# rakeshvar/theanet

Hardware: AMD Instinct MI355X
Metric: training images/sec (fwd+bwd+update) MNIST-CNN bs4096, 1/2/4/8 MI355X (higher is better)
Workload: dtype f32; 1 GPU; params/mnist.prms 28x28x1 synthetic, global batch 4096 = 4096 images/GPU/step x 1, elastic stage on; global_batch=4096, parallelism=dp1, schedule=two steps in flight (exact: the update applies the old velocity)

## Files before the change

theanet_amd/csrc/convblock_mfma.hip:

```cpp
#include "common.h"

int tn_conv_wgrad_finish(tn_ctx* ctx, const float* partial, const float* dbpartial, float* dW,
                         float* db, int nblk, int K, int C, int f);

typedef float f32x4 __attribute__((ext_vector_type(4)));

#define CM_XR 12

struct CmGeom {
    int N, H, Wd, K, pad, Ho, Wo, Hp, Wp;
    int Wx, xplane;
    int xf;
    int PT;
    int npixp;
    int dzf;
    int tabf;
    int wavef;
    int dbg;
};

__device__ __forceinline__ void cm_wave_sync() {
    __builtin_amdgcn_fence(__ATOMIC_ACQ_REL, "wavefront");
    __builtin_amdgcn_wave_barrier();
}

__device__ __forceinline__ f32x4 cm_mfma(float a, float b, f32x4 c) {
    return __builtin_amdgcn_mfma_f32_16x16x4f32(a, b, c, 0, 0, 0);
}

template <int N>
__device__ __forceinline__ float cm_shr(float v) {
    return __int_as_float(__builtin_amdgcn_update_dpp(0, __float_as_int(v), 0x110 + N, 0xf, 0xf, false));
}

__device__ __forceinline__ int cm_div(int n, float rd) { return __float2int_rz(((float)n + .5f) * rd); }

template <int ACT>
__device__ __forceinline__ float cm_act(float z, int act, float prm) {
    if (ACT == TN_ACT_LEAKY) return fmaxf(0.f, z) + fminf(0.f, z) * prm;
    return tn_act_fwd(z, act, prm);
}
template <int ACT>
__device__ __forceinline__ float cm_actg(float a, int act, float prm) {
    if (ACT == TN_ACT_LEAKY) return a > 0.f ? 1.f : (a < 0.f ? prm : (prm > 0.f ? 1.f + prm : 0.f));
    return tn_act_grad_from_out(a, act, prm);
}

template <int C, int KS2, int ACT>
__global__ __launch_bounds__(256, 2) void convblock_bwd_mfma(
    const float* __restrict__ x, const float* __restrict__ W, const float* __restrict__ b,
    const float* __restrict__ g, float* __restrict__ dx, float* __restrict__ partial,
    float* __restrict__ dbpartial, CmGeom q, int act, float prm, float* __restrict__ tdbg) {
    constexpr int F = 3, FF = 9, CKK = C * FF;
    constexpr int KS1 = (CKK + 3) / 4;
    constexpr int NT = (CKK + 16) / 16;
    constexpr int NKT = (KS2 + 3) / 4;
    constexpr int NTD = 3;
    extern __shared__ __attribute__((aligned(16))) float sm[];
    const int lane = threadIdx.x & 63, wv = threadIdx.x >> 6;
    const int lo = lane & 15, qd = lane >> 4;
    const long long t0_ = __builtin_readcyclecounter();
    int ts_ = 0;
#define CM_STAMP() if (tdbg && blockIdx.x == (q.dbg >> 8) && threadIdx.x == 0 && ts_ < 20) tdbg[ts_++] = (float)(__builtin_readcyclecounter() - t0_)
    const int K = q.K, HW = q.H * q.Wd, CHW = C * HW, HpWp = q.Hp * q.Wp, KHW = K * HpWp;

    const int gw = blockIdx.x * 4 + wv, nw = gridDim.x * 4;
    float xr[CM_XR], gr[CM_XR];
#define CM_PREFETCH(N_)                                                                     \
    {                                                                                       \
        const float* xp_ = x + (size_t)(N_) * CHW;                                          \
        const float* gp_ = g + (size_t)(N_) * KHW;                                          \
        _Pragma("unroll") for (int j = 0; j < CM_XR; ++j) {                                 \
            xr[j] = xp_[min(lane + 64 * j, CHW - 1)];                                       \
            gr[j] = gp_[min(lane + 64 * j, KHW - 1)];                                       \
        }                                                                                   \
    }
    int n = __builtin_amdgcn_readfirstlane(gw);
    if (n < q.N) CM_PREFETCH(n);

    int* wtab = reinterpret_cast<int*>(sm);
    float* wbase = sm + q.tabf + wv * q.wavef;
    float* sx = wbase;
    float* sdx = sx + q.xf;
    float* sg = sdx;
    float* sdz = sdx + q.xf;
    const int ZERO = q.xf - 4, ONE = q.xf - 3;
    const int DUMMY = q.xf - 2;

    for (int i = threadIdx.x; i < 4 * q.PT; i += 256) {
        int e = 0;
        if (i < HpWp) {
            const int wy = i / q.Wp, wx = i - wy * q.Wp;
            const bool vx = 2 * wx + 1 < q.Wo, vy = 2 * wy + 1 < q.Ho;
            e = ((2 * wy * q.Wx + 2 * wx) << 4) | 1 | (vx ? 2 : 0) | (vy ? 4 : 0) | (vx && vy ? 8 : 0);
        }
        wtab[i] = e;
    }
    for (int i = lane * 4; i < q.xf; i += 256) *reinterpret_cast<float4*>(sx + i) = make_float4(0.f, 0.f, 0.f, 0.f);
    for (int i = lane; i < 4 * KS2 * 4; i += 64) sdz[(i >> 2) * q.npixp + 16 * q.PT + (i & 3)] = 0.f;
    for (int i = K * q.npixp + lane; i < q.dzf; i += 64) sdz[i] = 0.f;
    CM_STAMP();
    __syncthreads();
    CM_STAMP();
    if (lane == 0) sx[ONE] = 1.f;

    auto ckk_off = [&](int ckk) {
        const int c = ckk / FF, ab = ckk - c * FF, a = ab / F, bb = ab - a * F;
        return c * q.xplane + a * q.Wx + bb;
    };
    auto wf = [&](int k, int c, int ab) -> float {
        const bool ok = k < K && c < C && ab < FF;
        const float v = W[((size_t)min(k, K - 1) * C + min(c, C - 1)) * FF + (FF - 1 - min(ab, FF - 1))];
        return ok ? v : 0.f;
    };
    float Bw1[NKT][KS1];
    int off1[KS1];
#pragma unroll
    for (int s = 0; s < KS1; ++s) {
        const int ckk = 4 * s + qd;
        off1[s] = ckk < CKK ? ckk_off(ckk) : 0;
#pragma unroll
        for (int kt = 0; kt < NKT; ++kt) Bw1[kt][s] = wf(16 * kt + lo, ckk < CKK ? ckk / FF : C, ckk % FF);
    }
    int off3[NT], msk3[NT];
#pragma unroll
    for (int nt = 0; nt < NT; ++nt) {
        const int ckk = 16 * nt + lo;
        off3[nt] = ckk < CKK ? ckk_off(ckk) : (ckk == CKK ? ONE : ZERO);
        msk3[nt] = ckk < CKK ? -1 : 0;
    }
    float Aw2[NTD][KS2];
#pragma unroll
    for (int mt = 0; mt < NTD; ++mt)
#pragma unroll
        for (int s = 0; s < KS2; ++s) Aw2[mt][s] = wf(4 * s + qd, lo >> 2, 4 * mt + (lo & 3));
    float bk[NKT];
#pragma unroll
    for (int kt = 0; kt < NKT; ++kt) bk[kt] = b[min(16 * kt + lo, K - 1)];
    int tabr[CM_XR];
    const float rHW = __builtin_amdgcn_rcpf((float)HW), rWd = __builtin_amdgcn_rcpf((float)q.Wd);
#pragma unroll
    for (int j = 0; j < CM_XR; ++j) {
        const int i = min(lane + 64 * j, CHW - 1);
        const int c = cm_div(i, rHW), r = i - c * HW, y = cm_div(r, rWd), xx = r - y * q.Wd;
        tabr[j] = (lane + 64 * j < CHW) ? c * q.xplane + (y + q.pad) * q.Wx + xx + q.pad : DUMMY;
    }
    CM_STAMP();
    __builtin_amdgcn_s_waitcnt(0x0f70);
    CM_STAMP();
#pragma unroll
    for (int s = 0; s < KS1; ++s)
#pragma unroll
        for (int kt = 0; kt < NKT; ++kt) asm volatile("" : "+v"(Bw1[kt][s]));
#pragma unroll
    for (int mt = 0; mt < NTD; ++mt)
#pragma unroll
        for (int s = 0; s < KS2; ++s) asm volatile("" : "+v"(Aw2[mt][s]));
#pragma unroll
    for (int kt = 0; kt < NKT; ++kt) asm volatile("" : "+v"(bk[kt]));

    f32x4 accW[NKT][NT];
#pragma unroll
    for (int kt = 0; kt < NKT; ++kt)
#pragma unroll
        for (int nt = 0; nt < NT; ++nt) accW[kt][nt] = f32x4{0.f, 0.f, 0.f, 0.f};
    CM_STAMP();

    const int dyo = ((lo >> 1) & 1) * q.Wx + (lo & 1);
    const float tie = prm > 0.f ? 1.f + prm : 0.f;
    const int dcol = lo < q.Wo ? 4 * (lo >> 1) + (lo & 1) : 16 * q.PT;
    const int dmsk = lo < q.Wo ? -1 : 0;
    for (; n < q.N; n += nw) {
#pragma unroll
        for (int j = 0; j < CM_XR; ++j) {
            sx[tabr[j]] = xr[j];
            sg[min(lane + 64 * j, KHW - 1)] = gr[j];
        }
        if (n + nw < q.N) CM_PREFETCH(n + nw);
        cm_wave_sync();
        CM_STAMP();
        float av[KS1];
        {
            const int poff = (wtab[lo >> 2] >> 4) + dyo;
#pragma unroll
            for (int s = 0; s < KS1; ++s) av[s] = sx[poff + off1[s]];
        }
#pragma unroll 1
        for (int t = 0; t < q.PT; ++t) {
            f32x4 z[NKT];
#pragma unroll
            for (int kt = 0; kt < NKT; ++kt) z[kt] = f32x4{0.f, 0.f, 0.f, 0.f};
            if (!(q.dbg & 8)) {
#pragma unroll
            for (int s = 0; s < KS1; ++s)
#pragma unroll
                for (int kt = 0; kt < NKT; ++kt) z[kt] = cm_mfma(av[s], Bw1[kt][s], z[kt]);
            }
            {
                const int tn = min(t + 1, q.PT - 1);
                const int poff = (wtab[4 * tn + (lo >> 2)] >> 4) + dyo;
#pragma unroll
                for (int s = 0; s < KS1; ++s) av[s] = sx[poff + off1[s]];
            }
            const int wi = 4 * t + qd;
            const int e2 = wtab[wi];
            const int woff = e2 >> 4;
            float bv[4][NT];
#pragma unroll
            for (int r = 0; r < 4; ++r) {
                const int pw = woff + (r >> 1) * q.Wx + (r & 1);
#pragma unroll
                for (int nt = 0; nt < NT; ++nt) bv[r][nt] = sx[off3[nt] + (pw & msk3[nt])];
            }
            float dzv[NKT][4];
#pragma unroll
            for (int kt = 0; kt < NKT; ++kt) {
                const int k = 16 * kt + lo;
                float gv = sg[min(k, K - 1) * HpWp + min(wi, HpWp - 1)];
                gv = k < K ? gv : 0.f;
                float a[4];
                float m = -INFINITY;
#pragma unroll
                for (int r = 0; r < 4; ++r) {
                    a[r] = cm_act<ACT>(z[kt][r] + bk[kt], act, prm);
                    m = (e2 >> r & 1) ? fmaxf(m, a[r]) : m;
                }
#pragma unroll
                for (int r = 0; r < 4; ++r) {
                    float gp;
                    if (ACT == TN_ACT_LEAKY) {
                        gp = a[r] < 0.f ? prm : tie;
                        gp = a[r] > 0.f ? 1.f : gp;
                    } else {
                        gp = tn_act_grad_from_out(a[r], act, prm);
                    }
                    const float sel = ((e2 >> r & 1) && a[r] == m) ? gv : 0.f;
                    dzv[kt][r] = sel * gp;
                }
                if (k < K)
                    *reinterpret_cast<float4*>(sdz + k * q.npixp + 16 * t + 4 * qd) =
                        make_float4(dzv[kt][0], dzv[kt][1], dzv[kt][2], dzv[kt][3]);
            }
            if (!(q.dbg & 1)) {
#pragma unroll
            for (int r = 0; r < 4; ++r)
#pragma unroll
                for (int kt = 0; kt < NKT; ++kt)
#pragma unroll
                    for (int nt = 0; nt < NT; ++nt)
                        accW[kt][nt] = cm_mfma(dzv[kt][r], bv[r][nt], accW[kt][nt]);
            }
        }
        CM_STAMP();
        if (dx && !(q.dbg & 2)) {
            cm_wave_sync();
            float R1 = 0.f, R2 = 0.f;
            float* dxo = sdx + qd * q.xplane + lo;
            const bool dlive = (qd < C) && (lo < q.Wo + 2);
            float bcur[KS2];
            {
                const float* dzp = sdz + qd * q.npixp + dcol;
#pragma unroll
                for (int s = 0; s < KS2; ++s) bcur[s] = dzp[4 * s * q.npixp];
            }
#pragma unroll 1
            for (int y = 0; y < q.Ho; ++y) {
                const int yn = min(y + 1, q.Ho - 1);
                const int prow = 4 * (yn >> 1) * q.Wp + 2 * (yn & 1);
                const float* dzp = sdz + qd * q.npixp + dcol + (prow & dmsk);
                float bnxt[KS2];
#pragma unroll
                for (int s = 0; s < KS2; ++s) bnxt[s] = dzp[4 * s * q.npixp];
                f32x4 T[NTD];
#pragma unroll
                for (int mt = 0; mt < NTD; ++mt) T[mt] = f32x4{0.f, 0.f, 0.f, 0.f};
#pragma unroll
                for (int s = 0; s < KS2; ++s)
#pragma unroll
                    for (int mt = 0; mt < NTD; ++mt) T[mt] = cm_mfma(Aw2[mt][s], bcur[s], T[mt]);
#pragma unroll
                for (int s = 0; s < KS2; ++s) bcur[s] = bnxt[s];
                const float S0 = T[0][0] + cm_shr<1>(T[0][1]) + cm_shr<2>(T[0][2]);
                const float S1 = T[0][3] + cm_shr<1>(T[1][0]) + cm_shr<2>(T[1][1]);
                const float S2 = T[1][2] + cm_shr<1>(T[1][3]) + cm_shr<2>(T[2][0]);
                const float out = S0 + R1;
                R1 = S1 + R2;
                R2 = S2;
                if (dlive) dxo[y * q.Wx] = out;
            }
            if (dlive) {
                dxo[q.Ho * q.Wx] = R1;
                dxo[(q.Ho + 1) * q.Wx] = R2;
            }
            cm_wave_sync();
            float* dxp = dx + (size_t)n * CHW;
#pragma unroll
            for (int j = 0; j < CM_XR; ++j) {
                const int i = lane + 64 * j;
                if (i < CHW) dxp[i] = sdx[tabr[j]];
            }
        }
        cm_wave_sync();
        CM_STAMP();
    }
#undef CM_PREFETCH
    __syncthreads();
#pragma unroll
    for (int kt = 0; kt < NKT; ++kt)
#pragma unroll
        for (int nt = 0; nt < NT; ++nt)
#pragma unroll
            for (int r = 0; r < 4; ++r) wbase[((kt * NT + nt) * 4 + r) * 64 + lane] = accW[kt][nt][r];
    __syncthreads();
    for (int e = threadIdx.x; e < K * (CKK + 1); e += 256) {
        const int k = e / (CKK + 1), ckk = e - k * (CKK + 1);
        const int idx = (((k >> 4) * NT + (ckk >> 4)) * 4 + (k & 3)) * 64 + ((k & 15) >> 2) * 16 + (ckk & 15);
        const float* src = sm + q.tabf + idx;
        const float s = ((src[0] + src[q.wavef]) + src[2 * q.wavef]) + src[3 * q.wavef];
        if (ckk < CKK)
            partial[(size_t)blockIdx.x * K * CKK + k * CKK + ckk] = s;
        else
            dbpartial[(size_t)blockIdx.x * K + k] = s;
    }
    CM_STAMP();
#undef CM_STAMP
}

template <int C, int KS2, int ACT, bool W44>
__global__ __launch_bounds__(256, 2) void convblock_bwd_mask_mfma(
    const float* __restrict__ x, const float* __restrict__ W, const float* __restrict__ g,
    const float* __restrict__ y, const uint8_t* __restrict__ mask, float* __restrict__ dx,
    float* __restrict__ partial, float* __restrict__ dbpartial, CmGeom q, int act, float prm,
    float* __restrict__ tdbg) {
    constexpr int F = 3, FF = 9, CKK = C * FF;
    constexpr int NKT = (KS2 + 3) / 4;
    constexpr int NT = (CKK + 16) / 16;
    constexpr int NTD = 3;
    extern __shared__ __attribute__((aligned(16))) float sm[];
    const int lane = threadIdx.x & 63, wv = threadIdx.x >> 6;
    const int lo = lane & 15, qd = lane >> 4;
    const long long t0_ = __builtin_readcyclecounter();
    int ts_ = 0;
#define CM_STAMP() if (tdbg && blockIdx.x == (q.dbg >> 8) && threadIdx.x == 0 && ts_ < 20) tdbg[ts_++] = (float)(__builtin_readcyclecounter() - t0_)
    const int K = q.K, HW = q.H * q.Wd, CHW = C * HW, HpWp = q.Hp * q.Wp, KHW = K * HpWp;

    const int gw = blockIdx.x * 4 + wv, nw = gridDim.x * 4;
    float xr[CM_XR], gr[CM_XR], yr[CM_XR];
    int mr[CM_XR];
#define CM_PREFETCH(N_)                                                                     \
    {                                                                                       \
        const float* xp_ = x + (size_t)(N_) * CHW;                                          \
        const float* gp_ = g + (size_t)(N_) * KHW;                                          \
        const float* yp_ = y + (size_t)(N_) * KHW;                                          \
        const uint8_t* mp_ = mask + (size_t)(N_) * KHW;                                     \
        _Pragma("unroll") for (int j = 0; j < CM_XR; ++j) {                                 \
            xr[j] = xp_[min(lane + 64 * j, CHW - 1)];                                       \
            gr[j] = gp_[min(lane + 64 * j, KHW - 1)];                                       \
            if (ACT != TN_ACT_LEAKY) yr[j] = yp_[min(lane + 64 * j, KHW - 1)];              \
            mr[j] = mp_[min(lane + 64 * j, KHW - 1)];                                       \
        }                                                                                   \
    }
    int n = __builtin_amdgcn_readfirstlane(gw);
    if (n < q.N) CM_PREFETCH(n);

    int* wtab = reinterpret_cast<int*>(sm);
    float* wbase = sm + q.tabf + wv * q.wavef;
    float* sx = wbase;
    float* sdx = sx + q.xf;
    float* sdz = sdx + q.xf;
    const int ZERO = q.xf - 4, ONE = q.xf - 3;
    const int DUMMY = q.xf - 2;

    for (int i = threadIdx.x; i < 4 * q.PT; i += 256) {
        const int w = min(i, HpWp - 1);
        const int wy = w / q.Wp, wx = w - wy * q.Wp;
        wtab[i] = 2 * wy * q.Wx + 2 * wx;
    }
    for (int i = lane * 4; i < q.xf; i += 256) *reinterpret_cast<float4*>(sx + i) = make_float4(0.f, 0.f, 0.f, 0.f);
    for (int i = lane * 4; i < q.dzf + 4; i += 256) *reinterpret_cast<float4*>(sdz + i) = make_float4(0.f, 0.f, 0.f, 0.f);
    __syncthreads();
    if (lane == 0) sx[ONE] = 1.f;

    auto ckk_off = [&](int ckk) {
        const int c = ckk / FF, ab = ckk - c * FF, a = ab / F, bb = ab - a * F;
        return c * q.xplane + a * q.Wx + bb;
    };
    int off3[NT], msk3[NT];
#pragma unroll
    for (int nt = 0; nt < NT; ++nt) {
        const int ckk = 16 * nt + lo;
        off3[nt] = ckk < CKK ? ckk_off(ckk) : (ckk == CKK ? ONE : ZERO);
        msk3[nt] = ckk < CKK ? -1 : 0;
    }
    int arow[NKT], amsk[NKT];
#pragma unroll
    for (int kt = 0; kt < NKT; ++kt) {
        const int k = 16 * kt + lo;
        arow[kt] = k < K ? k * q.npixp : q.dzf;
        amsk[kt] = k < K ? -1 : 0;
    }
    constexpr bool REM = CKK + 1 > 32;
    constexpr int NM = (KS2 + 1) / 2;
    const int g2 = lane >> 5, a8 = (lane >> 2) & 7, r4 = lane & 3, g8 = lane >> 3, a2 = (lane >> 2) & 1;
    const int fM = 4 * a8 + r4, tM = lane & 31, tR = 32 + 4 * a2 + r4;
    const int arowM = fM < K ? fM * q.npixp : q.dzf, amskM = fM < K ? -1 : 0;
    const int offM = tM < CKK ? ckk_off(min(tM, CKK - 1)) : (tM == CKK ? ONE : ZERO), mskM = tM < CKK ? -1 : 0;
    const int offR = tR < CKK ? ckk_off(min(tR, CKK - 1)) : (tR == CKK ? ONE : ZERO), mskR = tR < CKK ? -1 : 0;
    int arowR[NM], amskR[NM];
#pragma unroll
    for (int m = 0; m < NM; ++m) {
        const int f = 8 * m + 4 * a2 + r4;
        arowR[m] = f < K ? f * q.npixp : q.dzf;
        amskR[m] = f < K ? -1 : 0;
    }
    f32x4 accM[KS2], accR[KS2];
#pragma unroll
    for (int a_ = 0; a_ < KS2; ++a_) accM[a_] = accR[a_] = f32x4{0.f, 0.f, 0.f, 0.f};
    float Aw2[NTD][KS2];
#pragma unroll
    for (int mt = 0; mt < NTD; ++mt)
#pragma unroll
        for (int s = 0; s < KS2; ++s) {
            const int k = 4 * s + qd, c = lo >> 2, ab = 4 * mt + (lo & 3);
            const float v = W[((size_t)min(k, K - 1) * C + min(c, C - 1)) * FF + (FF - 1 - min(ab, FF - 1))];
            Aw2[mt][s] = (k < K && c < C && ab < FF) ? v : 0.f;
        }
    int tabr[CM_XR];
    int dzo[CM_XR];
    const float rHW = __builtin_amdgcn_rcpf((float)HW), rWd = __builtin_amdgcn_rcpf((float)q.Wd);
    const float rHpWp = __builtin_amdgcn_rcpf((float)HpWp);
#pragma unroll
    for (int j = 0; j < CM_XR; ++j) {
        const int i = min(lane + 64 * j, CHW - 1);
        const int c = cm_div(i, rHW), r = i - c * HW, yy = cm_div(r, rWd), xx = r - yy * q.Wd;
        tabr[j] = (lane + 64 * j < CHW) ? c * q.xplane + (yy + q.pad) * q.Wx + xx + q.pad : DUMMY;
        const int e = min(lane + 64 * j, KHW - 1);
        const int k = cm_div(e, rHpWp), w = e - k * HpWp;
        dzo[j] = k * q.npixp + 4 * w;
    }
    __builtin_amdgcn_s_waitcnt(0x0f70);
#pragma unroll
    for (int mt = 0; mt < NTD; ++mt)
#pragma unroll
        for (int s = 0; s < KS2; ++s) asm volatile("" : "+v"(Aw2[mt][s]));

    f32x4 accW[NKT][NT];
#pragma unroll
    for (int kt = 0; kt < NKT; ++kt)
#pragma unroll
        for (int nt = 0; nt < NT; ++nt) accW[kt][nt] = f32x4{0.f, 0.f, 0.f, 0.f};
    CM_STAMP();

    const float tie = prm > 0.f ? 1.f + prm : 0.f;
    const int dcol = lo < q.Wo ? 4 * (lo >> 1) + (lo & 1) : 16 * q.PT;
    const int dmsk = lo < q.Wo ? -1 : 0;
    for (; n < q.N; n += nw) {
#pragma unroll
        for (int j = 0; j < CM_XR; ++j) {
            sx[tabr[j]] = xr[j];
            const int m = mr[j];
            float gp;
            if (ACT == TN_ACT_LEAKY) {
                gp = (m & 32) ? prm : tie;
                gp = (m & 16) ? 1.f : gp;
            } else {
                gp = tn_act_grad_from_out(yr[j], act, prm);
            }
            const float gy = gr[j] * gp;
            *reinterpret_cast<float4*>(sdz + dzo[j]) =
                make_float4((m & 1) ? gy : 0.f, (m & 2) ? gy : 0.f, (m & 4) ? gy : 0.f, (m & 8) ? gy : 0.f);
        }
        if (n + nw < q.N) CM_PREFETCH(n + nw);
        cm_wave_sync();
        CM_STAMP();
        if constexpr (W44) {
            float4 a4c;
            float b4c[4], arc[NM], brc = 0.f;
#define CM_W4_LOAD(Q_, A_, B_, AR_, BR_)                                                    \
            {                                                                               \
                const int w_ = 2 * (Q_) + g2, wo_ = wtab[w_];                               \
                A_ = *reinterpret_cast<const float4*>(sdz + arowM + ((4 * w_) & amskM));    \
                _Pragma("unroll") for (int r = 0; r < 4; ++r)                               \
                    B_[r] = sx[offM + ((wo_ + (r >> 1) * q.Wx + (r & 1)) & mskM)];          \
                if (REM) {                                                                  \
                    const int wr_ = 2 * (Q_) + (g8 >> 2), er_ = g8 & 3;                     \
                    _Pragma("unroll") for (int m = 0; m < NM; ++m)                          \
                        AR_[m] = sdz[arowR[m] + ((4 * wr_ + er_) & amskR[m])];              \
                    BR_ = sx[offR + ((wtab[wr_] + (er_ >> 1) * q.Wx + (er_ & 1)) & mskR)];  \
                }                                                                           \
            }
            CM_W4_LOAD(0, a4c, b4c, arc, brc);
#pragma unroll 1
            for (int Q = 0; Q < 2 * q.PT; ++Q) {
                float4 a4n;
                float b4n[4], arn[NM], brn = 0.f;
                const int Qn = min(Q + 1, 2 * q.PT - 1);
                CM_W4_LOAD(Qn, a4n, b4n, arn, brn);
                if (!(q.dbg & 1)) {
#define CM_M4(AB) if (AB < KS2) accM[AB < KS2 ? AB : 0] = __builtin_amdgcn_mfma_f32_4x4x1f32(a_, b4c[s_], accM[AB < KS2 ? AB : 0], 3, AB, 0);
#pragma unroll
                    for (int s_ = 0; s_ < 4; ++s_) {
                        const float a_ = s_ == 0 ? a4c.x : s_ == 1 ? a4c.y : s_ == 2 ? a4c.z : a4c.w;
                        CM_M4(0) CM_M4(1) CM_M4(2) CM_M4(3) CM_M4(4) CM_M4(5) CM_M4(6) CM_M4(7)
                    }
#undef CM_M4
                    if (REM) {
#pragma unroll
                        for (int m = 0; m < NM; ++m) {
                            accR[2 * m] = __builtin_amdgcn_mfma_f32_4x4x1f32(arc[m], brc, accR[2 * m], 1, 0, 0);
                            if (2 * m + 1 < KS2)
                                accR[2 * m + 1 < KS2 ? 2 * m + 1 : 0] = __builtin_amdgcn_mfma_f32_4x4x1f32(
                                    arc[m], brc, accR[2 * m + 1 < KS2 ? 2 * m + 1 : 0], 1, 1, 0);
                        }
                    }
                }
                a4c = a4n;
#pragma unroll
                for (int r = 0; r < 4; ++r) b4c[r] = b4n[r];
#pragma unroll
                for (int m = 0; m < NM; ++m) arc[m] = arn[m];
                brc = brn;
            }
#undef CM_W4_LOAD
        } else {
        float4 ac[NKT];
        float bc[4][NT];
#define CM_WG_LOAD(T_, A_, B_)                                                              \
        {                                                                                   \
            const int po_ = 16 * (T_) + 4 * qd;                                             \
            _Pragma("unroll") for (int kt = 0; kt < NKT; ++kt)                              \
                A_[kt] = *reinterpret_cast<const float4*>(sdz + arow[kt] + (po_ & amsk[kt])); \
            const int wo_ = wtab[4 * (T_) + qd];                                            \
            _Pragma("unroll") for (int r = 0; r < 4; ++r) {                                 \
                const int pw_ = wo_ + (r >> 1) * q.Wx + (r & 1);                            \
                _Pragma("unroll") for (int nt = 0; nt < NT; ++nt)                           \
                    B_[r][nt] = sx[off3[nt] + (pw_ & msk3[nt])];                            \
            }                                                                               \
        }
        CM_WG_LOAD(0, ac, bc);
#pragma unroll 1
        for (int t = 0; t < q.PT; ++t) {
            float4 an[NKT];
            float bn[4][NT];
            const int tn = min(t + 1, q.PT - 1);
            CM_WG_LOAD(tn, an, bn);
            if (!(q.dbg & 1)) {
#pragma unroll
            for (int r = 0; r < 4; ++r)
#pragma unroll
                for (int kt = 0; kt < NKT; ++kt)
#pragma unroll
                    for (int nt = 0; nt < NT; ++nt) {
                        const float a = r == 0 ? ac[kt].x : r == 1 ? ac[kt].y : r == 2 ? ac[kt].z : ac[kt].w;
                        accW[kt][nt] = cm_mfma(a, bc[r][nt], accW[kt][nt]);
                    }
            }
#pragma unroll
            for (int kt = 0; kt < NKT; ++kt) ac[kt] = an[kt];
#pragma unroll
            for (int r = 0; r < 4; ++r)
#pragma unroll
                for (int nt = 0; nt < NT; ++nt) bc[r][nt] = bn[r][nt];
        }
#undef CM_WG_LOAD
        }
        CM_STAMP();
        if (dx && !(q.dbg & 2)) {
            float R1 = 0.f, R2 = 0.f;
            float* dxo = sdx + qd * q.xplane + lo;
            const bool dlive = (qd < C) && (lo < q.Wo + 2);
            float bcur[KS2];
            {
                const float* dzp = sdz + qd * q.npixp + dcol;
#pragma unroll
                for (int s = 0; s < KS2; ++s) bcur[s] = dzp[4 * s * q.npixp];
            }
#pragma unroll 1
            for (int yy = 0; yy < q.Ho; ++yy) {
                const int yn = min(yy + 1, q.Ho - 1);
                const int prow = 4 * (yn >> 1) * q.Wp + 2 * (yn & 1);
                const float* dzp = sdz + qd * q.npixp + dcol + (prow & dmsk);
                float bnxt[KS2];
#pragma unroll
                for (int s = 0; s < KS2; ++s) bnxt[s] = dzp[4 * s * q.npixp];
                f32x4 T[NTD];
#pragma unroll
                for (int mt = 0; mt < NTD; ++mt) T[mt] = f32x4{0.f, 0.f, 0.f, 0.f};
#pragma unroll
                for (int s = 0; s < KS2; ++s)
#pragma unroll
                    for (int mt = 0; mt < NTD; ++mt) T[mt] = cm_mfma(Aw2[mt][s], bcur[s], T[mt]);
#pragma unroll
                for (int s = 0; s < KS2; ++s) bcur[s] = bnxt[s];
                const float S0 = T[0][0] + cm_shr<1>(T[0][1]) + cm_shr<2>(T[0][2]);
                const float S1 = T[0][3] + cm_shr<1>(T[1][0]) + cm_shr<2>(T[1][1]);
                const float S2 = T[1][2] + cm_shr<1>(T[1][3]) + cm_shr<2>(T[2][0]);
                const float out = S0 + R1;
                R1 = S1 + R2;
                R2 = S2;
                if (dlive) dxo[yy * q.Wx] = out;
            }
            if (dlive) {
                dxo[q.Ho * q.Wx] = R1;
                dxo[(q.Ho + 1) * q.Wx] = R2;
            }
            cm_wave_sync();
            float* dxp = dx + (size_t)n * CHW;
#pragma unroll
            for (int j = 0; j < CM_XR; ++j) {
                const int i = lane + 64 * j;
                if (i < CHW) dxp[i] = sdx[tabr[j]];
            }
        }
        cm_wave_sync();
        CM_STAMP();
    }
#undef CM_PREFETCH
    __syncthreads();
    if constexpr (W44) {
#pragma unroll
        for (int a_ = 0; a_ < KS2; ++a_)
#pragma unroll
            for (int r = 0; r < 4; ++r) {
                wbase[(a_ * 4 + r) * 64 + lane] = accM[a_][r];
                if (REM) wbase[((KS2 + a_) * 4 + r) * 64 + lane] = accR[a_][r];
            }
        __syncthreads();
        for (int e = threadIdx.x; e < K * (CKK + 1); e += 256) {
            const int k = e / (CKK + 1), ckk = e - k * (CKK + 1);
            float s = 0.f;
            if (!REM || ckk < 32) {
                const float* src = sm + q.tabf + ((k >> 2) * 4 + (k & 3)) * 64 + ckk;
#pragma unroll
                for (int w = 0; w < 4; ++w) s += src[w * q.wavef] + src[w * q.wavef + 32];
            } else {
                const float* src = sm + q.tabf + ((KS2 + (k >> 2)) * 4 + (k & 3)) * 64 + (ckk - 32);
#pragma unroll
                for (int w = 0; w < 4; ++w) {
                    float t = 0.f;
#pragma unroll
                    for (int p8 = 0; p8 < 8; ++p8) t += src[w * q.wavef + 8 * p8];
                    s += t;
                }
            }
            if (ckk < CKK)
                partial[(size_t)blockIdx.x * K * CKK + k * CKK + ckk] = s;
            else
                dbpartial[(size_t)blockIdx.x * K + k] = s;
        }
    } else {
#pragma unroll
    for (int kt = 0; kt < NKT; ++kt)
#pragma unroll
        for (int nt = 0; nt < NT; ++nt)
#pragma unroll
            for (int r = 0; r < 4; ++r) wbase[((kt * NT + nt) * 4 + r) * 64 + lane] = accW[kt][nt][r];
    __syncthreads();
    for (int e = threadIdx.x; e < K * (CKK + 1); e += 256) {
        const int k = e / (CKK + 1), ckk = e - k * (CKK + 1);
        const int idx = (((k >> 4) * NT + (ckk >> 4)) * 4 + (k & 3)) * 64 + ((k & 15) >> 2) * 16 + (ckk & 15);
        const float* src = sm + q.tabf + idx;
        const float s = ((src[0] + src[q.wavef]) + src[2 * q.wavef]) + src[3 * q.wavef];
        if (ckk < CKK)
            partial[(size_t)blockIdx.x * K * CKK + k * CKK + ckk] = s;
        else
            dbpartial[(size_t)blockIdx.x * K + k] = s;
    }
    }
    CM_STAMP();
#undef CM_STAMP
}

static void cm_geometry(CmGeom& q, int C, int K) {
    q.Wx = q.Wo + 3;
    q.xplane = (q.Ho + 3) * q.Wx;
    q.xf = ((C * q.xplane + 3) & ~3) + 4;
    q.PT = (q.Hp * q.Wp + 3) / 4;
    q.npixp = 16 * q.PT + 4;
    q.dzf = 4 * ((K + 3) / 4) * q.npixp;
    q.tabf = (4 * q.PT + 3) & ~3;
    int red = 2 * ((C * 9 + 16) / 16) * 4 * 64;
    if (red < 2 * ((K + 3) / 4) * 4 * 64) red = 2 * ((K + 3) / 4) * 4 * 64;
    q.wavef = 2 * q.xf + q.dzf + 4;
    if (q.wavef < red) q.wavef = red;
}

static size_t cm_lds_bytes(const CmGeom& q) { return ((size_t)q.tabf + 4 * (size_t)q.wavef) * sizeof(float); }

static int cm_supported(int C, int K, int f, int stride, int p, int H, int Wd, int pad_lo, int Ho,
                        int Wo, int Hp, int Wp, bool recompute) {
    if (f != 3 || stride != 1 || p != 2 || C < 1 || C > 4 || K < 1 || K > 32) return 0;
    if (C * H * Wd > 64 * CM_XR || K * Hp * Wp > 64 * CM_XR) return 0;
    if (H + 2 * pad_lo > Ho + 2 || Wd + 2 * pad_lo > Wo + 2) return 0;
    if (Wo + 2 > 16) return 0;
    if (Hp != (Ho + 1) / 2 || Wp != (Wo + 1) / 2) return 0;
    CmGeom q;
    q.H = H; q.Wd = Wd; q.Ho = Ho; q.Wo = Wo; q.Hp = Hp; q.Wp = Wp; q.dbg = 0;
    cm_geometry(q, C, K);
    if (recompute && K * Hp * Wp > q.xf) return 0;
    return cm_lds_bytes(q) <= 78 * 1024;
}

int tn_convblock_mfma_supported(int C, int K, int f, int stride, int p, int H, int Wd, int pad_lo,
                                int Ho, int Wo, int Hp, int Wp) {
    return cm_supported(C, K, f, stride, p, H, Wd, pad_lo, Ho, Wo, Hp, Wp, true);
}

template <int C, int KS2>
static int launch_cm(tn_ctx* ctx, const float* x, const float* W, const float* b, const float* g,
                     float* dx, float* dW, float* db, CmGeom q, int act, float prm) {
    const size_t lds = cm_lds_bytes(q);
    int nblk = 2 * ctx->num_cus;
    if (nblk > cdiv(q.N, 4)) nblk = cdiv(q.N, 4);
    const size_t KCFF = (size_t)q.K * C * 9;
    float* partial;
    int rc = tn_scratch_get(ctx, (size_t)nblk * (KCFF + q.K) * sizeof(float), &partial);
    if (rc) return rc;
    float* dbpartial = partial + (size_t)nblk * KCFF;
    if (act == TN_ACT_LEAKY) {
        auto kern = convblock_bwd_mfma<C, KS2, TN_ACT_LEAKY>;
        static size_t set_for = 0;
        if (set_for < lds) {
            TN_HIP(hipFuncSetAttribute((const void*)kern, hipFuncAttributeMaxDynamicSharedMemorySize, (int)lds));
            set_for = lds;
        }
        kern<<<nblk, 256, lds, ctx->stream>>>(x, W, b, g, dx, partial, dbpartial, q, act, prm,
                                              (q.dbg & 16) ? db : nullptr);
    } else {
        auto kern = convblock_bwd_mfma<C, KS2, -1>;
        static size_t set_for = 0;
        if (set_for < lds) {
            TN_HIP(hipFuncSetAttribute((const void*)kern, hipFuncAttributeMaxDynamicSharedMemorySize, (int)lds));
            set_for = lds;
        }
        kern<<<nblk, 256, lds, ctx->stream>>>(x, W, b, g, dx, partial, dbpartial, q, act, prm,
                                              (q.dbg & 16) ? db : nullptr);
    }
    TN_LAUNCH_CHECK();
    if (q.dbg & 16) return TN_OK;
    return tn_conv_wgrad_finish(ctx, partial, dbpartial, dW, db, nblk, q.K, C, 3);
}

template <int C, int KS2>
static int launch_cm_mask(tn_ctx* ctx, const float* x, const float* W, const float* g, const float* y,
                          const uint8_t* mask, float* dx, float* dW, float* db, CmGeom q, int act,
                          float prm) {
    const size_t lds = cm_lds_bytes(q);
    int nblk = 2 * ctx->num_cus;
    if (nblk > cdiv(q.N, 4)) nblk = cdiv(q.N, 4);
    const size_t KCFF = (size_t)q.K * C * 9;
    float* partial;
    int rc = tn_scratch_get(ctx, (size_t)nblk * (KCFF + q.K) * sizeof(float), &partial);
    if (rc) return rc;
    float* dbpartial = partial + (size_t)nblk * KCFF;
    float* tdbg = (q.dbg & 16) ? db : nullptr;
    if (act == TN_ACT_LEAKY && tn_knob(TN_K_CB_W44)) {
        auto kern = convblock_bwd_mask_mfma<C, KS2, TN_ACT_LEAKY, true>;
        static size_t set_for = 0;
        if (set_for < lds) {
            TN_HIP(hipFuncSetAttribute((const void*)kern, hipFuncAttributeMaxDynamicSharedMemorySize, (int)lds));
            set_for = lds;
        }
        kern<<<nblk, 256, lds, ctx->stream>>>(x, W, g, y, mask, dx, partial, dbpartial, q, act, prm, tdbg);
    } else if (act == TN_ACT_LEAKY) {
        auto kern = convblock_bwd_mask_mfma<C, KS2, TN_ACT_LEAKY, false>;
        static size_t set_for = 0;
        if (set_for < lds) {
            TN_HIP(hipFuncSetAttribute((const void*)kern, hipFuncAttributeMaxDynamicSharedMemorySize, (int)lds));
            set_for = lds;
        }
        kern<<<nblk, 256, lds, ctx->stream>>>(x, W, g, y, mask, dx, partial, dbpartial, q, act, prm, tdbg);
    } else {
        auto kern = convblock_bwd_mask_mfma<C, KS2, -1, false>;
        static size_t set_for = 0;
        if (set_for < lds) {
            TN_HIP(hipFuncSetAttribute((const void*)kern, hipFuncAttributeMaxDynamicSharedMemorySize, (int)lds));
            set_for = lds;
        }
        kern<<<nblk, 256, lds, ctx->stream>>>(x, W, g, y, mask, dx, partial, dbpartial, q, act, prm, tdbg);
    }
    TN_LAUNCH_CHECK();
    if (q.dbg & 16) return TN_OK;
    return tn_conv_wgrad_finish(ctx, partial, dbpartial, dW, db, nblk, q.K, C, 3);
}

extern "C" int tn_convblock_mask_supported(int C, int K, int f, int stride, int p, int H, int Wd,
                                           int pad_lo, int Ho, int Wo, int Hp, int Wp) {
    return cm_supported(C, K, f, stride, p, H, Wd, pad_lo, Ho, Wo, Hp, Wp, false);
}

extern "C" int tn_convblock_bwd_mask(tn_ctx* ctx, const float* x, const float* W, const float* g,
                                     const float* y, const uint8_t* mask, float* dx, float* dW,
                                     float* db, int N, int C, int H, int Wd, int K, int f, int pad_lo,
                                     int Ho, int Wo, int p, int Hp, int Wp, int act, float act_param) {
    TN_REQUIRE(tn_convblock_mask_supported(C, K, f, 1, p, H, Wd, pad_lo, Ho, Wo, Hp, Wp),
               "tn_convblock_bwd_mask: unsupported C=%d K=%d f=%d p=%d %dx%d", C, K, f, p, H, Wd);
    TN_REQUIRE(x && W && g && y && mask && dW && db, "tn_convblock_bwd_mask: null argument");
    CmGeom q;
    q.N = N; q.H = H; q.Wd = Wd; q.K = K; q.pad = pad_lo; q.Ho = Ho; q.Wo = Wo; q.Hp = Hp; q.Wp = Wp;
    cm_geometry(q, C, K);
    q.dbg = tn_knob(TN_K_CM_DBG);
#define CM_KS(C_, S_) case S_: return launch_cm_mask<C_, S_>(ctx, x, W, g, y, mask, dx, dW, db, q, act, act_param)
#define CM_GO(C_)                                                                                  \
    switch ((K + 3) / 4) {                                                                         \
        CM_KS(C_, 1); CM_KS(C_, 2); CM_KS(C_, 3); CM_KS(C_, 4);                                    \
        CM_KS(C_, 5); CM_KS(C_, 6); CM_KS(C_, 7); default: CM_KS(C_, 8);                           \
    }
    switch (C) {
        case 1: CM_GO(1);
        case 2: CM_GO(2);
        case 3: CM_GO(3);
        default: CM_GO(4);
    }
#undef CM_GO
#undef CM_KS
}

int tn_convblock_mfma_bwd(tn_ctx* ctx, const float* x, const float* W, const float* b, const float* g,
                          float* dx, float* dW, float* db, int N, int C, int H, int Wd, int K,
                          int pad_lo, int Ho, int Wo, int Hp, int Wp, int act, float act_param) {
    CmGeom q;
    q.N = N; q.H = H; q.Wd = Wd; q.K = K; q.pad = pad_lo; q.Ho = Ho; q.Wo = Wo; q.Hp = Hp; q.Wp = Wp;
    cm_geometry(q, C, K);
    q.dbg = tn_knob(TN_K_CM_DBG);
#define CM_KS(C_, S_) case S_: return launch_cm<C_, S_>(ctx, x, W, b, g, dx, dW, db, q, act, act_param)
#define CM_GO(C_)                                                                                  \
    switch ((K + 3) / 4) {                                                                         \
        CM_KS(C_, 1); CM_KS(C_, 2); CM_KS(C_, 3); CM_KS(C_, 4);                                    \
        CM_KS(C_, 5); CM_KS(C_, 6); CM_KS(C_, 7); default: CM_KS(C_, 8);                           \
    }
    switch (C) {
        case 1: CM_GO(1);
        case 2: CM_GO(2);
        case 3: CM_GO(3);
        default: CM_GO(4);
    }
#undef CM_GO
#undef CM_KS
}
```

Before: 24.61 million images/sec.

## Restructure conv backward MFMA loops with byte-offset LDS addressing and two-stage unrolling

Rewrites the 4x4 weight-gradient inner loop to unroll by two with ping-pong register buffers. Addresses are now precomputed byte offsets into LDS that advance incrementally, replacing the per-iteration mask and table arithmetic. The dgrad row loop gets the same double-buffered unroll with sched barriers, and the dz masking uses bitfield-extract ANDs instead of selects. The intent is to cut VALU address overhead and hide LDS latency behind the MFMAs, at the cost of more registers and more subtle edge handling (changed ONE/DUMMY slots, bound_ctrl DPP, padding reads that are no longer clamped).

```diff
diff --git a/theanet_amd/csrc/convblock_mfma.hip b/theanet_amd/csrc/convblock_mfma.hip
--- a/theanet_amd/csrc/convblock_mfma.hip
+++ b/theanet_amd/csrc/convblock_mfma.hip
@@ -31,6 +31,18 @@
 template <int N>
 __device__ __forceinline__ float cm_shr(float v) {
     return __int_as_float(__builtin_amdgcn_update_dpp(0, __float_as_int(v), 0x110 + N, 0xf, 0xf, false));
+}
+
+template <int N>
+__device__ __forceinline__ float cm_shrz(float v) {
+    return __int_as_float(__builtin_amdgcn_update_dpp(0, __float_as_int(v), 0x110 + N, 0xf, 0xf, true));
+}
+
+template <int B>
+__device__ __forceinline__ float cm_bit_and(int m, float v) {
+    int s;
+    asm("v_bfe_i32 %0, %1, %2, 1" : "=v"(s) : "v"(m), "n"(B));
+    return __int_as_float(s & __float_as_int(v));
 }
 
 __device__ __forceinline__ int cm_div(int n, float rd) { return __float2int_rz(((float)n + .5f) * rd); }
@@ -368,18 +380,17 @@
     float* sx = wbase;
     float* sdx = sx + q.xf;
     float* sdz = sdx + q.xf;
-    const int ZERO = q.xf - 4, ONE = q.xf - 3;
-    const int DUMMY = q.xf - 2;
+    const int ZERO = q.xf - 4, ONE = q.xf - 2;
 
     for (int i = threadIdx.x; i < 4 * q.PT; i += 256) {
         const int w = min(i, HpWp - 1);
         const int wy = w / q.Wp, wx = w - wy * q.Wp;
-        wtab[i] = 2 * wy * q.Wx + 2 * wx;
+        wtab[i] = (2 * wy * q.Wx + 2 * wx) * (W44 ? 4 : 1);
     }
     for (int i = lane * 4; i < q.xf; i += 256) *reinterpret_cast<float4*>(sx + i) = make_float4(0.f, 0.f, 0.f, 0.f);
     for (int i = lane * 4; i < q.dzf + 4; i += 256) *reinterpret_cast<float4*>(sdz + i) = make_float4(0.f, 0.f, 0.f, 0.f);
     __syncthreads();
-    if (lane == 0) sx[ONE] = 1.f;
+    if (lane < 2) sx[ONE + lane] = 1.f;
 
     auto ckk_off = [&](int ckk) {
         const int c = ckk / FF, ab = ckk - c * FF, a = ab / F, bb = ab - a * F;
@@ -403,15 +414,28 @@
     constexpr int NM = (KS2 + 1) / 2;
     const int g2 = lane >> 5, a8 = (lane >> 2) & 7, r4 = lane & 3, g8 = lane >> 3, a2 = (lane >> 2) & 1;
     const int fM = 4 * a8 + r4, tM = lane & 31, tR = 32 + 4 * a2 + r4;
-    const int arowM = fM < K ? fM * q.npixp : q.dzf, amskM = fM < K ? -1 : 0;
-    const int offM = tM < CKK ? ckk_off(min(tM, CKK - 1)) : (tM == CKK ? ONE : ZERO), mskM = tM < CKK ? -1 : 0;
-    const int offR = tR < CKK ? ckk_off(min(tR, CKK - 1)) : (tR == CKK ? ONE : ZERO), mskR = tR < CKK ? -1 : 0;
-    int arowR[NM], amskR[NM];
-#pragma unroll
-    for (int m = 0; m < NM; ++m) {
-        const int f = 8 * m + 4 * a2 + r4;
-        arowR[m] = f < K ? f * q.npixp : q.dzf;
-        amskR[m] = f < K ? -1 : 0;
+    const int offM = tM < CKK ? ckk_off(min(tM, CKK - 1)) : (tM == CKK ? ONE : ZERO);
+    const int offR = tR < CKK ? ckk_off(min(tR, CKK - 1)) : (tR == CKK ? ONE : ZERO);
+    const int er4 = g8 & 3;
+    const char* const smb = reinterpret_cast<const char*>(sm);
+    const int sxo = 4 * (q.tabf + wv * q.wavef), sdzo = sxo + 8 * q.xf;
+    constexpr bool ALLM = CKK >= 32;
+    int oA = sdzo + 4 * (min(fM, 4 * KS2 - 1) * q.npixp + 4 * g2);
+    const int oBt = sxo + 4 * offM;
+    const int oBb = sxo + 4 * (offM + (tM < CKK ? q.Wx : 0));
+    const int mulM = tM < CKK ? 1 : 0;
+    const int oBR = sxo + 4 * (offR + (tR < CKK ? (er4 >> 1) * q.Wx + (er4 & 1) : 0));
+    int mulR = tR < CKK ? 1 : 0;
+    asm volatile("" : "+v"(mulR));
+    int oAR[NM];
+#pragma unroll
+    for (int m = 0; m < NM; ++m)
+        oAR[m] = sdzo + 4 * (min(8 * m + 4 * a2 + r4, 4 * KS2 - 1) * q.npixp + 4 * g2 + er4);
+    const int oTab = 4 * g2;
+    if (W44) {
+        asm volatile("" : "+v"(oA));
+#pragma unroll
+        for (int m = 0; m < NM; ++m) asm volatile("" : "+v"(oAR[m]));
     }
     f32x4 accM[KS2], accR[KS2];
 #pragma unroll
@@ -433,7 +457,7 @@
     for (int j = 0; j < CM_XR; ++j) {
         const int i = min(lane + 64 * j, CHW - 1);
         const int c = cm_div(i, rHW), r = i - c * HW, yy = cm_div(r, rWd), xx = r - yy * q.Wd;
-        tabr[j] = (lane + 64 * j < CHW) ? c * q.xplane + (yy + q.pad) * q.Wx + xx + q.pad : DUMMY;
+        tabr[j] = c * q.xplane + (yy + q.pad) * q.Wx + xx + q.pad;
         const int e = min(lane + 64 * j, KHW - 1);
         const int k = cm_div(e, rHpWp), w = e - k * HpWp;
         dzo[j] = k * q.npixp + 4 * w;
@@ -453,7 +477,8 @@
 
     const float tie = prm > 0.f ? 1.f + prm : 0.f;
     const int dcol = lo < q.Wo ? 4 * (lo >> 1) + (lo & 1) : 16 * q.PT;
-    const int dmsk = lo < q.Wo ? -1 : 0;
+    const int oD = sdzo + 4 * (qd * q.npixp + dcol);
+    const int incD = lo < q.Wo ? 16 * q.Wp : 0;
     for (; n < q.N; n += nw) {
 #pragma unroll
         for (int j = 0; j < CM_XR; ++j) {
@@ -468,60 +493,68 @@
             }
             const float gy = gr[j] * gp;
             *reinterpret_cast<float4*>(sdz + dzo[j]) =
-                make_float4((m & 1) ? gy : 0.f, (m & 2) ? gy : 0.f, (m & 4) ? gy : 0.f, (m & 8) ? gy : 0.f);
+                make_float4(cm_bit_and<0>(m, gy), cm_bit_and<1>(m, gy), cm_bit_and<2>(m, gy), cm_bit_and<3>(m, gy));
         }
         if (n + nw < q.N) CM_PREFETCH(n + nw);
         cm_wave_sync();
         CM_STAMP();
         if constexpr (W44) {
-            float4 a4c;
-            float b4c[4], arc[NM], brc = 0.f;
-#define CM_W4_LOAD(Q_, A_, B_, AR_, BR_)                                                    \
-            {                                                                               \
-                const int w_ = 2 * (Q_) + g2, wo_ = wtab[w_];                               \
-                A_ = *reinterpret_cast<const float4*>(sdz + arowM + ((4 * w_) & amskM));    \
-                _Pragma("unroll") for (int r = 0; r < 4; ++r)                               \
-                    B_[r] = sx[offM + ((wo_ + (r >> 1) * q.Wx + (r & 1)) & mskM)];          \
-                if (REM) {                                                                  \
-                    const int wr_ = 2 * (Q_) + (g8 >> 2), er_ = g8 & 3;                     \
-                    _Pragma("unroll") for (int m = 0; m < NM; ++m)                          \
-                        AR_[m] = sdz[arowR[m] + ((4 * wr_ + er_) & amskR[m])];              \
-                    BR_ = sx[offR + ((wtab[wr_] + (er_ >> 1) * q.Wx + (er_ & 1)) & mskR)];  \
-                }                                                                           \
-            }
-            CM_W4_LOAD(0, a4c, b4c, arc, brc);
+            float4 a4[2];
+            float b4[2][4], ar[2][NM], br[2] = {0.f, 0.f};
+#define CM_W4_TAB(Q_) (*reinterpret_cast<const int*>(smb + oTab + 8 * (Q_)))
+#define CM_W4_LOAD(OFF_, S_, WO_)                                                                           \
+            {                                                                                               \
+                a4[S_] = *reinterpret_cast<const float4*>(smb + oA + (OFF_));                               \
+                const int wm_ = ALLM ? (WO_) : __mul24((WO_), mulM);                                        \
+                const float* t_ = reinterpret_cast<const float*>(smb + oBt + wm_);                          \
+                const float* u_ = reinterpret_cast<const float*>(smb + oBb + wm_);                          \
+                b4[S_][0] = t_[0]; b4[S_][1] = t_[1]; b4[S_][2] = u_[0]; b4[S_][3] = u_[1];                 \
+                if (REM) {                                                                                  \
+                    _Pragma("unroll") for (int m = 0; m < NM; ++m)                                          \
+                        ar[S_][m] = *reinterpret_cast<const float*>(smb + oAR[m] + (OFF_));                 \
+                    br[S_] = *reinterpret_cast<const float*>(smb + oBR + __mul24((WO_), mulR));             \
+                }                                                                                           \
+            }
+#define CM_M4(S_, AB) if (AB < KS2) accM[AB < KS2 ? AB : 0] = __builtin_amdgcn_mfma_f32_4x4x1f32(a_, b4[S_][s_], accM[AB < KS2 ? AB : 0], 3, AB, 0);
+#define CM_W4_PRODUCTS(S_)                                                                                  \
+            if (!nowg) {                                                                                    \
+                _Pragma("unroll") for (int s_ = 0; s_ < 4; ++s_) {                                          \
+                    const float a_ = s_ == 0 ? a4[S_].x : s_ == 1 ? a4[S_].y : s_ == 2 ? a4[S_].z : a4[S_].w; \
+                    CM_M4(S_, 0) CM_M4(S_, 1) CM_M4(S_, 2) CM_M4(S_, 3) CM_M4(S_, 4) CM_M4(S_, 5) CM_M4(S_, 6) CM_M4(S_, 7) \
+                }                                                                                           \
+                if (REM) {                                                                                  \
+                    _Pragma("unroll") for (int m = 0; m < NM; ++m) {                                        \
+                        accR[2 * m] = __builtin_amdgcn_mfma_f32_4x4x1f32(ar[S_][m], br[S_], accR[2 * m], 1, 0, 0); \
+                        if (2 * m + 1 < KS2)                                                                \
+                            accR[2 * m + 1 < KS2 ? 2 * m + 1 : 0] = __builtin_amdgcn_mfma_f32_4x4x1f32(     \
+                                ar[S_][m], br[S_], accR[2 * m + 1 < KS2 ? 2 * m + 1 : 0], 1, 1, 0);         \
+                    }                                                                                       \
+                }                                                                                           \
+            }
+            const int QL = 2 * q.PT - 1;
+            const int nowg = __builtin_amdgcn_readfirstlane(q.dbg & 1);
+            int woE = CM_W4_TAB(0), woO = CM_W4_TAB(1);
+            CM_W4_LOAD(0, 0, woE);
+            woE = CM_W4_TAB(min(2, QL));
 #pragma unroll 1
-            for (int Q = 0; Q < 2 * q.PT; ++Q) {
-                float4 a4n;
-                float b4n[4], arn[NM], brn = 0.f;
-                const int Qn = min(Q + 1, 2 * q.PT - 1);
-                CM_W4_LOAD(Qn, a4n, b4n, arn, brn);
-                if (!(q.dbg & 1)) {
-#define CM_M4(AB) if (AB < KS2) accM[AB < KS2 ? AB : 0] = __builtin_amdgcn_mfma_f32_4x4x1f32(a_, b4c[s_], accM[AB < KS2 ? AB : 0], 3, AB, 0);
-#pragma unroll
-                    for (int s_ = 0; s_ < 4; ++s_) {
-                        const float a_ = s_ == 0 ? a4c.x : s_ == 1 ? a4c.y : s_ == 2 ? a4c.z : a4c.w;
-                        CM_M4(0) CM_M4(1) CM_M4(2) CM_M4(3) CM_M4(4) CM_M4(5) CM_M4(6) CM_M4(7)
-                    }
+            for (int Q = 0; Q < QL; Q += 2) {
+                CM_W4_LOAD(32, 1, woO);
+                woO = CM_W4_TAB(min(Q + 3, QL));
+                CM_W4_PRODUCTS(0);
+                CM_W4_LOAD(64, 0, woE);
+                woE = CM_W4_TAB(min(Q + 4, QL));
+                CM_W4_PRODUCTS(1);
+                oA += 64;
+#pragma unroll
+                for (int m = 0; m < NM; ++m) oAR[m] += 64;
+            }
+            oA -= 64 * q.PT;
+#pragma unroll
+            for (int m = 0; m < NM; ++m) oAR[m] -= 64 * q.PT;
+#undef CM_W4_PRODUCTS
 #undef CM_M4
-                    if (REM) {
-#pragma unroll
-                        for (int m = 0; m < NM; ++m) {
-                            accR[2 * m] = __builtin_amdgcn_mfma_f32_4x4x1f32(arc[m], brc, accR[2 * m], 1, 0, 0);
-                            if (2 * m + 1 < KS2)
-                                accR[2 * m + 1 < KS2 ? 2 * m + 1 : 0] = __builtin_amdgcn_mfma_f32_4x4x1f32(
-                                    arc[m], brc, accR[2 * m + 1 < KS2 ? 2 * m + 1 : 0], 1, 1, 0);
-                        }
-                    }
-                }
-                a4c = a4n;
-#pragma unroll
-                for (int r = 0; r < 4; ++r) b4c[r] = b4n[r];
-#pragma unroll
-                for (int m = 0; m < NM; ++m) arc[m] = arn[m];
-                brc = brn;
-            }
 #undef CM_W4_LOAD
+#undef CM_W4_TAB
         } else {
         float4 ac[NKT];
         float bc[4][NT];
@@ -569,47 +602,57 @@
             float R1 = 0.f, R2 = 0.f;
             float* dxo = sdx + qd * q.xplane + lo;
             const bool dlive = (qd < C) && (lo < q.Wo + 2);
-            float bcur[KS2];
-            {
-                const float* dzp = sdz + qd * q.npixp + dcol;
-#pragma unroll
-                for (int s = 0; s < KS2; ++s) bcur[s] = dzp[4 * s * q.npixp];
-            }
+            float bE[KS2], bO[KS2];
+#define CM_DG_LOAD(B_, T_, OFF_)                                                                            \
+            {                                                                                               \
+                const char* p_ = smb + oD + __mul24((T_), incD) + (OFF_);                                   \
+                _Pragma("unroll") for (int s = 0; s < KS2; ++s)                                             \
+                    B_[s] = *reinterpret_cast<const float*>(p_ + s * (16 * q.npixp));                       \
+            }
+#define CM_DG_ROW(B_, YY_)                                                                                  \
+            {                                                                                               \
+                f32x4 T[NTD];                                                                               \
+                _Pragma("unroll") for (int mt = 0; mt < NTD; ++mt) T[mt] = f32x4{0.f, 0.f, 0.f, 0.f};       \
+                _Pragma("unroll") for (int s = 0; s < KS2; ++s)                                             \
+                    _Pragma("unroll") for (int mt = 0; mt < NTD; ++mt) T[mt] = cm_mfma(Aw2[mt][s], B_[s], T[mt]); \
+                const float S0 = T[0][0] + cm_shrz<1>(T[0][1]) + cm_shrz<2>(T[0][2]);                       \
+                const float S1 = T[0][3] + cm_shrz<1>(T[1][0]) + cm_shrz<2>(T[1][1]);                       \
+                const float S2 = T[1][2] + cm_shrz<1>(T[1][3]) + cm_shrz<2>(T[2][0]);                       \
+                const float out = S0 + R1;                                                                  \
+                R1 = S1 + R2;                                                                               \
+                R2 = S2;                                                                                    \
+                if (dlive) dxo[(YY_) * q.Wx] = out;                                                         \
+            }
+            const int TL = (q.Ho - 1) >> 1;
+            CM_DG_LOAD(bE, 0, 0);
 #pragma unroll 1
-            for (int yy = 0; yy < q.Ho; ++yy) {
-                const int yn = min(yy + 1, q.Ho - 1);
-                const int prow = 4 * (yn >> 1) * q.Wp + 2 * (yn & 1);
-                const float* dzp = sdz + qd * q.npixp + dcol + (prow & dmsk);
-                float bnxt[KS2];
-#pragma unroll
-                for (int s = 0; s < KS2; ++s) bnxt[s] = dzp[4 * s * q.npixp];
-                f32x4 T[NTD];
-#pragma unroll
-                for (int mt = 0; mt < NTD; ++mt) T[mt] = f32x4{0.f, 0.f, 0.f, 0.f};
-#pragma unroll
-                for (int s = 0; s < KS2; ++s)
-#pragma unroll
-                    for (int mt = 0; mt < NTD; ++mt) T[mt] = cm_mfma(Aw2[mt][s], bcur[s], T[mt]);
-#pragma unroll
-                for (int s = 0; s < KS2; ++s) bcur[s] = bnxt[s];
-                const float S0 = T[0][0] + cm_shr<1>(T[0][1]) + cm_shr<2>(T[0][2]);
-                const float S1 = T[0][3] + cm_shr<1>(T[1][0]) + cm_shr<2>(T[1][1]);
-                const float S2 = T[1][2] + cm_shr<1>(T[1][3]) + cm_shr<2>(T[2][0]);
-                const float out = S0 + R1;
-                R1 = S1 + R2;
-                R2 = S2;
-                if (dlive) dxo[yy * q.Wx] = out;
-            }
+            for (int t = 0; t < (q.Ho >> 1); ++t) {
+                CM_DG_LOAD(bO, t, 8);
+                __builtin_amdgcn_sched_barrier(0);
+                CM_DG_ROW(bE, 2 * t);
+                CM_DG_LOAD(bE, min(t + 1, TL), 0);
+                __builtin_amdgcn_sched_barrier(0);
+                CM_DG_ROW(bO, 2 * t + 1);
+            }
+            if (q.Ho & 1) CM_DG_ROW(bE, q.Ho - 1);
+#undef CM_DG_ROW
+#undef CM_DG_LOAD
             if (dlive) {
                 dxo[q.Ho * q.Wx] = R1;
                 dxo[(q.Ho + 1) * q.Wx] = R2;
             }
             cm_wave_sync();
+            CM_STAMP();
             float* dxp = dx + (size_t)n * CHW;
+            float dv[CM_XR];
+#pragma unroll
+            for (int j = 0; j < CM_XR; ++j) dv[j] = sdx[tabr[j]];
+#pragma unroll
+            for (int j = 0; j < CM_XR; ++j) asm volatile("" : "+v"(dv[j]));
 #pragma unroll
             for (int j = 0; j < CM_XR; ++j) {
                 const int i = lane + 64 * j;
-                if (i < CHW) dxp[i] = sdx[tabr[j]];
+                if (i < CHW) dxp[i] = dv[j];
             }
         }
         cm_wave_sync();
```

Result: faster. 24.94 million images/sec (median of 6 runs) (+1.3%).
